# FauxFaux/quadrs

Hardware: AMD Instinct MI355X
Metric: Msamples/s through shift->FIR->FFT chain (higher is better)
Workload: dtype f32

## Files before the change

### quadrs_amd/csrc/qd_chain.h

```cpp
#pragma once

#include "qd_device.h"
#include "qd_geometry.h"

namespace qd {

#ifdef QD_STAMP
#define QD_STAMP_DECL unsigned long long st_prev = 0, st_acc[8] = {0, 0, 0, 0, 0, 0, 0, 0}, st_row[4] = {0, 0, 0, 0}; unsigned st_tiles = 0;
#define QD_STAMP_ROW(k) do { unsigned long long t_; asm volatile("s_memtime %0\n\ts_waitcnt lgkmcnt(0)" : "=s"(t_) :: "memory"); st_row[k] += t_ - st_prev; st_acc[0] += t_ - st_prev; st_prev = t_; } while (0)
#define QD_STAMP_START() do { asm volatile("s_memtime %0\n\ts_waitcnt lgkmcnt(0)" : "=s"(st_prev) :: "memory"); } while (0)
#define QD_STAMP_AT(k) do { unsigned long long t_; asm volatile("s_memtime %0\n\ts_waitcnt lgkmcnt(0)" : "=s"(t_) :: "memory"); st_acc[k] += t_ - st_prev; st_prev = t_; } while (0)
#define QD_STAMP_FLUSH() do { if (P.stamps && (threadIdx.x & 63) == 0 && threadIdx.x < 1024) { unsigned w_ = threadIdx.x >> 6; for (int k_ = 0; k_ < 8; ++k_) atomicAdd(&P.stamps[w_ * 8 + k_], st_acc[k_]); if (w_ == 1) for (int k_ = 0; k_ < 4; ++k_) atomicAdd(&P.stamps[129 + k_], st_row[k_]); if (w_ == 0) for (int k_ = 0; k_ < 4; ++k_) atomicAdd(&P.stamps[133 + k_], st_row[k_]); if (w_ == 0) atomicAdd(&P.stamps[128], (unsigned long long)st_tiles); } } while (0)
#define QD_STAMP_TILE() do { ++st_tiles; } while (0)
#else
#define QD_STAMP_DECL
#define QD_STAMP_START()
#define QD_STAMP_AT(k)
#define QD_STAMP_FLUSH()
#define QD_STAMP_TILE()
#define QD_STAMP_ROW(k)
#endif

#ifdef QD_DEVELOP
#define QD_DBG(P, bit) (((P).dbg & (bit)) != 0)
// ... 535 lines not shown
        }
    };
    auto load_h1 = [&](uint32_t j0, float *hh) {
        const float4 *hp = reinterpret_cast<const float4 *>(h + j0);
#pragma unroll
        for (int v = 0; v < BS / 4; ++v) {
            const float4 q = hp[v];
            hh[4 * v + 0] = q.x; hh[4 * v + 1] = q.y; hh[4 * v + 2] = q.z; hh[4 * v + 3] = q.w;
        }
    };
    auto load_h = [&](uint32_t blk, float (*hh)[BS]) {
#pragma unroll
        for (int r = 0; r < R; ++r) load_h1(blk * BS - r * D, hh[r]);
    };
    bool lane_trunc = false;
#pragma unroll
    for (int r = 0; r < R; ++r) lane_trunc |= jmax[r] < T;
    const bool need_snap = __builtin_amdgcn_ballot_w64(lane_trunc) != 0;
    auto snap_check = [&](int r, uint32_t j0) {
        if (need_snap && j0 >= T / 2 + D && ((j0 - T / 2) % D) == 0) {
            if (jmax[r] == j0) { sr[r] = ar[r]; si[r] = ai[r]; }
        }
    };
    auto mac_int = [&](uint32_t blk, const float2 *x, const float (*hh)[BS]) {
#pragma unroll
        for (int r = 0; r < R; ++r) snap_check(r, blk * BS - r * D);
#pragma unroll
        for (int i = 0; i < BS; ++i) {
#pragma unroll
            for (int r = 0; r < R; ++r) {
                ar[r] = ar[r] + x[i].x * hh[r][i];
                ai[r] = ai[r] + x[i].y * hh[r][i];
            }
        }
    };
    auto mac_edge = [&](uint32_t blk, const float2 *x) {
#pragma unroll
        for (int r = 0; r < R; ++r) {
            const int32_t j0 = (int32_t)(blk * BS) - r * (int32_t)D;
            if (j0 >= 0 && j0 < (int32_t)T) {
                snap_check(r, (uint32_t)j0);
                float hh[BS];
                load_h1((uint32_t)j0, hh);
#pragma unroll
                for (int i = 0; i < BS; ++i) {
                    ar[r] = ar[r] + x[i].x * hh[i];
                    ai[r] = ai[r] + x[i].y * hh[i];
                }
            }
        }
    };
    constexpr uint32_t P = (R - 1) * D / BS, E = T / BS;
    static_assert(E > P + 2, "filter too short for the register-tiled FIR");
    constexpr uint32_t P2 = P + ((E - P) & 1);
    float2 xa[BS], xb[BS];
    float ha[R][BS], hb[R][BS];
#pragma unroll
    for (uint32_t blk = 0; blk < P2; ++blk) {
        load_x(blk, xa);
        if (blk < P) mac_edge(blk, xa); else { load_h(blk, ha); mac_int(blk, xa, ha); }
    }
    load_x(P2, xa); load_h(P2, ha);
    for (uint32_t blk = P2; blk + 2 < E; blk += 2) {
        load_x(blk + 1, xb); load_h(blk + 1, hb);
        mac_int(blk, xa, ha);
        __builtin_amdgcn_sched_barrier(0);
        load_x(blk + 2, xa); load_h(blk + 2, ha);
        mac_int(blk + 1, xb, hb);
        __builtin_amdgcn_sched_barrier(0);
    }
    load_x(E - 1, xb); load_h(E - 1, hb);
    mac_int(E - 2, xa, ha);
    load_x(E, xa);
    mac_int(E - 1, xb, hb);
#pragma unroll
    for (uint32_t blk = E; blk < NB; ++blk) {
        if (blk > E) load_x(blk, xa);
        mac_edge(blk, xa);
    }
#pragma unroll
    for (int r = 0; r < R; ++r) { full[r] = make_float2(ar[r], ai[r]); snap[r] = make_float2(sr[r], si[r]); }
}

template <class GeoT>
__device__ __forceinline__ float fir_comp(const float *xp, uint32_t jmax, const float *h, float *snap_out = nullptr) {
    constexpr uint32_t D = GeoT::D, Dp = GeoT::Dp, T = GeoT::T, b = GeoT::b0;
    constexpr uint32_t PRE = (8 - b % 8) % 8, NBLK = (T - PRE) / 8, TAIL = (T - PRE) % 8;
    constexpr uint32_t CPOS = (T / 2 + 8 * D - PRE) % 8;
    static_assert(D % 8 == 0 && NBLK >= 3, "component-split FIR geometry");
    float acc = 0.f, snap = 0.f;
    auto cand = [&](uint32_t jj) -> bool { return jj >= T / 2 + D && jj < T && ((jj - T / 2) % D) == 0; };
    auto xoff = [&](uint32_t t) -> uint32_t { return 2 * ((t / D) * Dp + (t % D)); };
#pragma unroll
    for (uint32_t i = 0; i < PRE; ++i) {
        if (cand(i)) { if (jmax == i) snap = acc; }
        acc = acc + xp[xoff(b + i)] * h[i];
    }
    float xa[8], xb[8], ha[8], hb[8];
    auto load = [&](uint32_t m, float *x, float *hh) {
        const uint32_t t = b + PRE + 8 * m;
        const float *pp = xp + xoff(t);
#pragma unroll
        for (int i = 0; i < 8; ++i) x[i] = pp[2 * i];
        if constexpr (PRE % 4 == 0) {
            const float4 *hp = reinterpret_cast<const float4 *>(h + PRE + 8 * m);
            const float4 h0 = hp[0], h1 = hp[1];
            hh[0] = h0.x; hh[1] = h0.y; hh[2] = h0.z; hh[3] = h0.w; hh[4] = h1.x; hh[5] = h1.y; hh[6] = h1.z; hh[7] = h1.w;
        } else {
#pragma unroll
            for (int i = 0; i < 8; ++i) hh[i] = h[PRE + 8 * m + i];
        }
    };
    auto mac = [&](uint32_t m, const float *x, const float *hh) {
#pragma unroll
        for (uint32_t i = 0; i < 8; ++i) {
            if (i == CPOS) { const uint32_t jj = PRE + 8 * m + i; if (cand(jj) && jmax == jj) snap = acc; }
            acc = acc + x[i] * hh[i];
        }
    };
    constexpr uint32_t NPAIR = NBLK / 2;
    load(0, xa, ha);
    auto pair = [&](uint32_t m) {
        load(m + 1, xb, hb);
        mac(m, xa, ha);
        asm volatile("" : "+v"(acc));
        __builtin_amdgcn_sched_barrier(0);
        load(m + 2, xa, ha);
        mac(m + 1, xb, hb);
        asm volatile("" : "+v"(acc));
        __builtin_amdgcn_sched_barrier(0);
    };
    if constexpr (NPAIR <= 16) {
#pragma unroll
        for (uint32_t m = 0; m + 2 < 2 * NPAIR; m += 2) pair(m);
    } else {
#pragma unroll 1
        for (uint32_t m = 0; m + 2 < 2 * NPAIR; m += 2) pair(m);
    }
    load(2 * NPAIR - 1, xb, hb);
    mac(2 * NPAIR - 2, xa, ha);
    if constexpr (NBLK % 2) load(NBLK - 1, xa, ha);
    mac(2 * NPAIR - 1, xb, hb);
    if constexpr (NBLK % 2) mac(NBLK - 1, xa, ha);
#pragma unroll
    for (uint32_t i = 0; i < TAIL; ++i) {
        const uint32_t jj = PRE + 8 * NBLK + i;
        if (cand(jj)) { if (jmax == jj) snap = acc; }
        acc = acc + xp[xoff(b + jj)] * h[jj];
    }
    if (snap_out) { *snap_out = snap; return acc; }
    return jmax < T ? snap : acc;
}

template <class GeoT>
__device__ __forceinline__ float2 fir_pair(const float2 *rowp , uint32_t jmax, const float *h, float2 *snap_out = nullptr) {
    constexpr uint32_t D = GeoT::D, Dp = GeoT::Dp, T = GeoT::T, b = GeoT::b0, NB = T / 4;
    constexpr int PF = 3;
    static_assert(GeoT::kPad == 2 && T % 4 == 0 && b % 2 == 0 && D % 4 == 0 && NB > (uint32_t)PF, "packed FIR geometry");
#if defined(QD_FIR_ABL) && (QD_FIR_ABL & 4)
    if (snap_out) *snap_out = rowp[1];
    return rowp[0];
#endif
    v2f acc = {0.f, 0.f}, snap = {0.f, 0.f};
    auto cand = [&](uint32_t jj) -> bool { return jj >= T / 2 + D && jj < T && ((jj - T / 2) % D) == 0; };
    auto xoff = [&](uint32_t t) -> uint32_t { return (t / D) * Dp + (t % D); };
    float4 xa[PF], xb[PF], hh[PF];
    auto load = [&](uint32_t k, int slot) {
        const uint32_t t0 = b + 4 * k;
        xa[slot] = *reinterpret_cast<const float4 *>(rowp + xoff(t0));
        xb[slot] = *reinterpret_cast<const float4 *>(rowp + xoff(t0 + 2));
        hh[slot] = *reinterpret_cast<const float4 *>(h + 4 * k);
    };
#pragma unroll
    for (int k = 0; k < PF; ++k) load(k, k);
#pragma unroll
    for (uint32_t k = 0; k < NB; ++k) {
        const int slot = (int)(k % PF);
        if (cand(4 * k)) { if (jmax == 4 * k) snap = acc; }
        static_assert((T / 2) % 4 == 0, "snapshot taps sit on block boundaries");
        const v2f x0 = {xa[slot].x, xa[slot].y}, x1 = {xa[slot].z, xa[slot].w}, x2 = {xb[slot].x, xb[slot].y}, x3 = {xb[slot].z, xb[slot].w};
        const v2f h01 = {hh[slot].x, hh[slot].y}, h23 = {hh[slot].z, hh[slot].w};
        v2f p0, p1;
        if constexpr ((GeoT::kFlags & kGeoFastFma) != 0) {
            asm volatile("v_pk_fma_f32 %0, %1, %5, %0 op_sel_hi:[1,0,1]\n\t"
                         "v_pk_fma_f32 %0, %2, %5, %0 op_sel:[0,1,0] op_sel_hi:[1,1,1]\n\t"
                         "v_pk_fma_f32 %0, %3, %6, %0 op_sel_hi:[1,0,1]\n\t"
                         "v_pk_fma_f32 %0, %4, %6, %0 op_sel:[0,1,0] op_sel_hi:[1,1,1]"
                         : "+v"(acc)
                         : "v"(x0), "v"(x1), "v"(x2), "v"(x3), "v"(h01), "v"(h23));
        } else
        asm volatile("v_pk_mul_f32 %1, %3, %7 op_sel_hi:[1,0]\n\t"
                     "v_pk_mul_f32 %2, %4, %7 op_sel:[0,1] op_sel_hi:[1,1]\n\t"
                     "v_pk_add_f32 %0, %0, %1\n\t"
                     "v_pk_mul_f32 %1, %5, %8 op_sel_hi:[1,0]\n\t"
                     "v_pk_add_f32 %0, %0, %2\n\t"
                     "v_pk_mul_f32 %2, %6, %8 op_sel:[0,1] op_sel_hi:[1,1]\n\t"
                     "v_pk_add_f32 %0, %0, %1\n\t"
                     "v_pk_add_f32 %0, %0, %2"
                     : "+v"(acc), "=&v"(p0), "=&v"(p1)
                     : "v"(x0), "v"(x1), "v"(x2), "v"(x3), "v"(h01), "v"(h23));
        if (k + PF < NB) load(k + PF, slot);
        __builtin_amdgcn_sched_barrier(0);
    }
    if (snap_out) { *snap_out = make_float2(snap.x, snap.y); return make_float2(acc.x, acc.y); }
    const v2f r = jmax < T ? snap : acc;
    return make_float2(r.x, r.y);
}

template <class GeoT, int TURN>
__device__ __forceinline__ void fir_tiled2_pk(const float2 *lanep, const float *h, float2 *full, const uint32_t *jm, float2 *snap) {
    constexpr uint32_t D = GeoT::D, T = GeoT::T, c = GeoT::c;
    constexpr uint32_t L = D + T, NB = L / 4, HB = T / 4, LAG = D / 4;
    constexpr bool kReTap = LAG > 4;
    constexpr int PF = 3, NS = kReTap ? PF : PF + (int)LAG + 1;

    static_assert(GeoT::kFirTile == 2 && GeoT::PD == 2 * D && GeoT::pshift != 0xffffffffu && GeoT::kPad == 2, "two-output packed FIR: layout");
    static_assert(D % 4 == 0 && T % 4 == 0 && c % 4 == 0 && (T / 2) % 4 == 0 && NB > (uint32_t)PF && LAG >= 1 && LAG <= 8, "two-output packed FIR: geometry");
    v2f a0 = {0.f, 0.f}, a1 = {0.f, 0.f}, s0 = {0.f, 0.f}, s1 = {0.f, 0.f};
    const bool need_snap = __builtin_amdgcn_ballot_w64(jm[0] < T || jm[1] < T) != 0;
    auto cand = [&](uint32_t j) -> bool { return j >= T / 2 + D && j < T && ((j - T / 2) % D) == 0; };
    float4 xa[PF], xb[PF], hh[NS], gg[kReTap ? PF : 1];
    typedef float f4n __attribute__((ext_vector_type(4)));
    typedef __attribute__((address_space(3))) const f4n lds_f4;
    uint32_t hbase = (uint32_t)(uintptr_t)(__attribute__((address_space(3))) const void *)h;
    asm volatile("" : "+v"(hbase));
    const lds_f4 *hl = (const lds_f4 *)(uintptr_t)hbase;
    auto load = [&](uint32_t b) {
#if defined(QD_FIR_ABL) && (QD_FIR_ABL & 2)
        if (b >= (uint32_t)PF) return;
#endif
        const uint32_t t = c + 4 * b;
        const float2 *pp = lanep + (t + GeoT::kPad * (t >> GeoT::pshift));
        xa[b % PF] = *reinterpret_cast<const float4 *>(pp);
        xb[b % PF] = *reinterpret_cast<const float4 *>(pp + 2);
        if (b < HB) { const f4n q = hl[b]; hh[b % NS] = make_float4(q.x, q.y, q.z, q.w); }
        if constexpr (kReTap) { if (b >= LAG) { const f4n q = hl[b - LAG]; gg[b % PF] = make_float4(q.x, q.y, q.z, q.w); } }
    };
#pragma unroll
    for (int b = 0; b < PF; ++b) load(b);
#pragma clang loop unroll(full)
    for (uint32_t b = 0; b < NB; ++b) {
        const float4 A = xa[b % PF], B = xb[b % PF];
        const v2f x0 = {A.x, A.y}, x1 = {A.z, A.w}, x2 = {B.x, B.y}, x3 = {B.z, B.w};
        v2f t0, t1, t2, t3;
        if constexpr (TURN >= 0) { if ((b % 8) == 0) { if (((b / 8) & 1u) != (uint32_t)TURN) __builtin_amdgcn_s_setprio(2); else __builtin_amdgcn_s_setprio(1); } }
        if ((b < HB && cand(4 * b)) || (b >= LAG && cand(4 * (b - LAG)))) {
            if (need_snap) {
                if (b < HB && cand(4 * b)) { if (jm[0] == 4 * b) s0 = a0; }
                if (b >= LAG && cand(4 * (b - LAG))) { if (jm[1] == 4 * (b - LAG)) s1 = a1; }
            }
        }
#if defined(QD_FIR_ABL) && (QD_FIR_ABL & 1)
        {
            asm volatile("" :: "v"(x0), "v"(x3), "v"(hh[b % NS].x));
            if (b + PF < NB) load(b + PF);
            __builtin_amdgcn_sched_barrier(0);
            continue;
        }
#endif
        if (b >= LAG && b < HB) {
            const float4 H = hh[b % NS], G = kReTap ? gg[b % PF] : hh[(b - LAG) % NS];
            const v2f h01 = {H.x, H.y}, h23 = {H.z, H.w}, g01 = {G.x, G.y}, g23 = {G.z, G.w};
            if constexpr ((GeoT::kFlags & kGeoFastFma) != 0) {
                asm volatile("v_pk_fma_f32 %0, %2, %6, %0 op_sel_hi:[1,0,1]\n\t"
                             "v_pk_fma_f32 %1, %2, %8, %1 op_sel_hi:[1,0,1]\n\t"
                             "v_pk_fma_f32 %0, %3, %6, %0 op_sel:[0,1,0] op_sel_hi:[1,1,1]\n\t"
                             "v_pk_fma_f32 %1, %3, %8, %1 op_sel:[0,1,0] op_sel_hi:[1,1,1]\n\t"
                             "v_pk_fma_f32 %0, %4, %7, %0 op_sel_hi:[1,0,1]\n\t"
                             "v_pk_fma_f32 %1, %4, %9, %1 op_sel_hi:[1,0,1]\n\t"
                             "v_pk_fma_f32 %0, %5, %7, %0 op_sel:[0,1,0] op_sel_hi:[1,1,1]\n\t"
                             "v_pk_fma_f32 %1, %5, %9, %1 op_sel:[0,1,0] op_sel_hi:[1,1,1]"
                             : "+v"(a0), "+v"(a1)
                             : "v"(x0), "v"(x1), "v"(x2), "v"(x3), "v"(h01), "v"(h23), "v"(g01), "v"(g23));
            } else
            asm volatile("v_pk_mul_f32 %2, %6, %10 op_sel_hi:[1,0]\n\t"
                         "v_pk_mul_f32 %3, %6, %12 op_sel_hi:[1,0]\n\t"
                         "v_pk_mul_f32 %4, %7, %10 op_sel:[0,1] op_sel_hi:[1,1]\n\t"
                         "v_pk_add_f32 %0, %0, %2\n\t"
                         "v_pk_mul_f32 %5, %7, %12 op_sel:[0,1] op_sel_hi:[1,1]\n\t"
                         "v_pk_add_f32 %1, %1, %3\n\t"
                         "v_pk_mul_f32 %2, %8, %11 op_sel_hi:[1,0]\n\t"
                         "v_pk_add_f32 %0, %0, %4\n\t"
                         "v_pk_mul_f32 %3, %8, %13 op_sel_hi:[1,0]\n\t"
                         "v_pk_add_f32 %1, %1, %5\n\t"
                         "v_pk_mul_f32 %4, %9, %11 op_sel:[0,1] op_sel_hi:[1,1]\n\t"
                         "v_pk_add_f32 %0, %0, %2\n\t"
                         "v_pk_mul_f32 %5, %9, %13 op_sel:[0,1] op_sel_hi:[1,1]\n\t"
                         "v_pk_add_f32 %1, %1, %3\n\t"
                         "v_pk_add_f32 %0, %0, %4\n\t"
                         "v_pk_add_f32 %1, %1, %5"
                         : "+v"(a0), "+v"(a1), "=&v"(t0), "=&v"(t1), "=&v"(t2), "=&v"(t3)
                         : "v"(x0), "v"(x1), "v"(x2), "v"(x3), "v"(h01), "v"(h23), "v"(g01), "v"(g23));
        } else {
            const float4 H = b < HB ? hh[b % NS] : (kReTap ? gg[b % PF] : hh[(b - LAG) % NS]);
            const v2f h01 = {H.x, H.y}, h23 = {H.z, H.w};
            v2f &acc = b < HB ? a0 : a1;
            if constexpr ((GeoT::kFlags & kGeoFastFma) != 0) {
                asm volatile("v_pk_fma_f32 %0, %1, %5, %0 op_sel_hi:[1,0,1]\n\t"
                             "v_pk_fma_f32 %0, %2, %5, %0 op_sel:[0,1,0] op_sel_hi:[1,1,1]\n\t"
                             "v_pk_fma_f32 %0, %3, %6, %0 op_sel_hi:[1,0,1]\n\t"
                             "v_pk_fma_f32 %0, %4, %6, %0 op_sel:[0,1,0] op_sel_hi:[1,1,1]"
                             : "+v"(acc)
                             : "v"(x0), "v"(x1), "v"(x2), "v"(x3), "v"(h01), "v"(h23));
            } else
            asm volatile("v_pk_mul_f32 %1, %3, %7 op_sel_hi:[1,0]\n\t"
                         "v_pk_mul_f32 %2, %4, %7 op_sel:[0,1] op_sel_hi:[1,1]\n\t"
                         "v_pk_add_f32 %0, %0, %1\n\t"
                         "v_pk_mul_f32 %1, %5, %8 op_sel_hi:[1,0]\n\t"
                         "v_pk_add_f32 %0, %0, %2\n\t"
                         "v_pk_mul_f32 %2, %6, %8 op_sel:[0,1] op_sel_hi:[1,1]\n\t"
                         "v_pk_add_f32 %0, %0, %1\n\t"
                         "v_pk_add_f32 %0, %0, %2"
                         : "+v"(acc), "=&v"(t0), "=&v"(t1)
                         : "v"(x0), "v"(x1), "v"(x2), "v"(x3), "v"(h01), "v"(h23));
        }
        if (b + PF < NB) load(b + PF);
        __builtin_amdgcn_sched_barrier(0);
    }
    full[0] = make_float2(a0.x, a0.y);
    full[1] = make_float2(a1.x, a1.y);
    snap[0] = make_float2(s0.x, s0.y);
    snap[1] = make_float2(s1.x, s1.y);
}

template <class GeoT>
__device__ __forceinline__ float2 fir_prefix(const float2 *raw, uint32_t t0, uint32_t jmax, const float *h) {
    constexpr uint32_t T = GeoT::T;
    float ar = 0.f, ai = 0.f;
    uint32_t jhi = jmax;
#pragma unroll
    for (int off = 32; off >= 1; off >>= 1) { const uint32_t o = (uint32_t)__shfl_xor((int)jhi, off); jhi = o > jhi ? o : jhi; }
// ... 1165 lines not shown
template <> struct SparkSwz<8, 4> { static constexpr uint32_t m[4] = {0x50, 0x20, 0x0, 0x0}; };
template <> struct SparkSwz<64, 1> { static constexpr uint32_t m[4] = {0x40, 0x90, 0x20, 0x40}; };
template <> struct SparkSwz<128, 1> { static constexpr uint32_t m[4] = {0x8, 0x10, 0x20, 0x40}; };
template <> struct SparkSwz<32, 1> { static constexpr uint32_t m[4] = {0x8, 0x10, 0x20, 0x40}; };
template <> struct SparkSwz<16, 1> { static constexpr uint32_t m[4] = {0x10, 0x20, 0x40, 0x80}; };
template <> struct SparkSwz<256, 1> { static constexpr uint32_t m[4] = {0x40, 0x90, 0x20, 0x40}; };
template <class SZ> struct SparkSwzFn {
    static constexpr uint32_t mask_off(uint32_t off) {
        uint32_t r = 0;
        for (uint32_t d = 1; d <= 4; ++d) if ((SZ::m[d - 1] >> (d + off)) & 1u) r |= 1u << d;
        return r;
    }
    static __device__ __forceinline__ constexpr uint32_t delta(uint32_t p) {
        constexpr uint32_t k1 = mask_off(1), k2 = mask_off(2), k3 = mask_off(3), k4 = mask_off(4), k5 = mask_off(5), k6 = mask_off(6), k7 = mask_off(7), k8 = mask_off(8);
        return ((p >> 1) & k1) ^ ((p >> 2) & k2) ^ ((p >> 3) & k3) ^ ((p >> 4) & k4) ^ ((p >> 5) & k5) ^ ((p >> 6) & k6) ^ ((p >> 7) & k7) ^ ((p >> 8) & k8);
    }
};

typedef float spark_f2n __attribute__((ext_vector_type(2)));
typedef float spark_f4n __attribute__((ext_vector_type(4)));
typedef __attribute__((address_space(3))) spark_f2n spark_lds_f2;
typedef __attribute__((address_space(3))) spark_f4n spark_lds_f4;
__device__ __forceinline__ float2 spark_ld2(uint32_t a) { const spark_f2n v = *(const spark_lds_f2 *)(uintptr_t)a; return make_float2(v.x, v.y); }
__device__ __forceinline__ void spark_st2(uint32_t a, float2 v) { *(spark_lds_f2 *)(uintptr_t)a = spark_f2n{v.x, v.y}; }

template <class GeoT, uint32_t TS, uint32_t SPL, int PART = 3 , bool RT = false >
__device__ __forceinline__ void spark_fft_swz(const ChainParams &P, const float2 *twl, uint32_t fb , uint32_t lane_in,
                                              uint32_t n_win = TS / GeoT::W) {
    using SZ = SparkSwzFn<SparkSwz<GeoT::W, SPL>>;
    constexpr uint32_t base = GeoT::base_len, lb = GeoT::log_base, layers = GeoT::layers;
    static_assert(base == 8 || base == 16, "spark_fft_swz: W >= 8");
    uint32_t lo = lane_in;
    asm volatile("" : "+v"(lo));
    auto wsync = [] { __builtin_amdgcn_fence(__ATOMIC_ACQ_REL, "wavefront"); __builtin_amdgcn_wave_barrier(); };
    constexpr uint32_t n_task = TS / base;
    const uint32_t n_task_rt = n_win << (GeoT::logW - lb);
    if constexpr ((PART & 1) != 0) {
#pragma unroll
    for (uint32_t k = 0; k < (n_task + 63) / 64; ++k) {
        const uint32_t t = lo + 64 * k;
        if (RT ? t < n_task_rt : (n_task % 64 == 0 || t < n_task)) {
            const uint32_t r0 = t << lb, a0 = fb + ((r0 ^ SZ::delta(r0)) << 3);
            float2 v[base];
#pragma unroll
            for (uint32_t q = 0; q < base / 2; ++q) {
                const spark_f4n pc = *(const spark_lds_f4 *)(uintptr_t)(a0 ^ (16 * q));
                v[2 * q] = make_float2(pc.x, pc.y); v[2 * q + 1] = make_float2(pc.z, pc.w);
            }
            if constexpr (base == 16) bf16(v, P.tw16_1, P.tw16_2, P.tw16_3, P.root2); else bf8(v, P.root2);
            uint32_t a1 = a0;
            asm volatile("" : "+v"(a1));
#pragma unroll
            for (uint32_t q = 0; q < base / 2; ++q)
                *(spark_lds_f4 *)(uintptr_t)(a1 ^ (16 * q)) = spark_f4n{v[2 * q].x, v[2 * q].y, v[2 * q + 1].x, v[2 * q + 1].y};
        }
    }
    }
    uint32_t cols = base, log_cols = lb, tw_off = 0;
    const uint32_t n_bf_rt = n_win << (GeoT::logW - 2);
    if constexpr ((PART & 2) != 0) {
#pragma unroll
    for (uint32_t l = 0; l < layers; ++l) {
        wsync();
        float2 tc1 = make_float2(0.f, 0.f), tc2 = tc1, tc3 = tc1;
        if (cols <= 64) { const uint32_t i = lo & (cols - 1); tc1 = twl[tw_off + 3 * i]; tc2 = twl[tw_off + 3 * i + 1]; tc3 = twl[tw_off + 3 * i + 2]; }
#pragma unroll
        for (uint32_t k = 0; k < (TS / 4 + 63) / 64; ++k) {
            const uint32_t t = lo + 64 * k, chunk = t >> log_cols, i = t & (cols - 1);
            if (RT ? t >= n_bf_rt : ((TS / 4) % 64 != 0 && t >= TS / 4)) continue;
            const uint32_t p0 = chunk * 4 * cols + i, b0 = fb + ((p0 ^ SZ::delta(p0)) << 3);
            uint32_t dp[4];
#pragma unroll
            for (uint32_t q = 0; q < 4; ++q) {
                const uint32_t qc = q * cols, lo_q = (qc ^ SZ::delta(qc)) & 31u, hi_q = qc & ~31u;
                dp[q] = (b0 ^ (lo_q << 3)) + (hi_q << 3);
            }
            float2 t1 = tc1, t2 = tc2, t3 = tc3;
            if (cols > 64) { t1 = twl[tw_off + 3 * i]; t2 = twl[tw_off + 3 * i + 1]; t3 = twl[tw_off + 3 * i + 2]; }
            float2 s0 = spark_ld2(dp[0]);
            float2 s1 = cmul(spark_ld2(dp[1]), t1);
            float2 s2 = cmul(spark_ld2(dp[2]), t2);
            float2 s3 = cmul(spark_ld2(dp[3]), t3);
            bf4(s0, s1, s2, s3);
            spark_st2(dp[0], s0); spark_st2(dp[1], s1); spark_st2(dp[2], s2); spark_st2(dp[3], s3);
        }
        tw_off += 3 * cols; cols *= 4; log_cols += 2;
    }
    }
    wsync();
}


template <int FMT, class GeoT, int PT_ = kPipe3Prod>
struct Pipe3S {
    static_assert(PT_ == 256 || PT_ == 512, "producer threads: 256 or 512");
    static constexpr Pipe3sRules K = pipe3s_rules(FmtTraits<FMT>::SPL, PT_, GeoT::R);
    static constexpr uint32_t SPL = K.SPL, ROW = K.ROW;
    static constexpr uint32_t W = GeoT::W, S = GeoT::S, D = GeoT::D, T = GeoT::T, G = GeoT::G, Dp = GeoT::Dp;
    static constexpr uint32_t N = K.N, RN = K.RN, GS = K.GS;
    static constexpr uint32_t c_half = GeoT::c, ntrunc = GeoT::kNtrunc;
    static constexpr uint32_t f0 = K.f0, RR = K.RR, RINGD = K.RINGD, MIRD = K.MIRD, ROWP = K.ROWP, RAW_ELEMS = K.RAW_ELEMS, DR = K.DR;
    static constexpr bool kOverlap = K.kOverlap, fir_ok = K.fir_ok, ok = K.ok, kWrite = K.kWrite;
    static_assert(!kWrite || !kOverlap, "the write sink's sub-blocks lie side by side");
    static constexpr uint32_t FBX_OFF = K.FBX_OFF, kLdsBytes = K.kLdsBytes;
    static constexpr uint32_t GH = K.GH;
    static constexpr bool kSwzFft = K.kSwzFft;
    static constexpr uint32_t kConsumerThreads = K.kConsumerThreads;
};

template <int FMT, int NCO, class GeoT, int RN_, int LB, int PT_ = kPipe3Prod>
__global__ __launch_bounds__(PT_ + ((GeoT::kFlags & kGeoWriteSink) ? 256 : 512), LB) void k_chain_pipe3s(const ChainParams P) {
    static_assert((GeoT::kFlags & kGeoWindow) == 0, "kGeoWindow: only k_chain applies the plan's window; this kernel would ignore it");
    using FT = FmtTraits<FMT>;
    using Vec = typename FT::Vec;
    using K = Pipe3S<FMT, GeoT, PT_>;
    constexpr int SPL = FT::SPL;
    constexpr bool HAS_SHIFT = NCO != 0;
    static_assert(K::ok && (uint32_t)RN_ == K::RN, "streaming three-stage kernel: geometry");
    constexpr bool kWrite = K::kWrite;
    constexpr uint32_t PT = PT_, NTHR = PT_ + K::kConsumerThreads, PW = PT_ / 64;
    constexpr uint32_t W = K::W, S = K::S, D = K::D, T = K::T, G = K::G, Dp = K::Dp, logW = GeoT::logW;
    constexpr uint32_t ROW = K::ROW, ROWB = ROW * FT::BPS, VECB = SPL * FT::BPS, RN = K::RN, RR = K::RR, GS = K::GS, DR = K::DR;
    const GeoT geo(P);

    extern __shared__ __attribute__((aligned(16))) char smem[];
    float2 *raw = reinterpret_cast<float2 *>(smem);
    float2 *dec = raw + K::RAW_ELEMS, *trc = dec + DR;
    float2 *fbx = raw + K::FBX_OFF;
    float2 *twl = fbx + 2 * (size_t)G * W;
    float *tapl = reinterpret_cast<float *>(kWrite ? raw + K::RAW_ELEMS : twl + W);
    if (P.lds_dyn < K::kLdsBytes) return;

    const uint32_t tid = threadIdx.x;
    const uint32_t wave = __builtin_amdgcn_readfirstlane(tid >> 6);
    {
        if constexpr (!kWrite) {
            const uint32_t n_tw = W - geo.base_len;
            for (uint32_t i = tid; i < n_tw; i += NTHR) twl[i] = P.tw[i];
        }
        for (uint32_t i = tid; i < T; i += NTHR) tapl[i] = P.taps[i];
    }
    __syncthreads();

    const uint64_t n_tiles = (P.n_windows + G - 1) / G;
    const uint64_t base_cnt = n_tiles / gridDim.x, rem = n_tiles % gridDim.x;
    const uint64_t t_lo = (uint64_t)blockIdx.x * base_cnt + (blockIdx.x < rem ? blockIdx.x : rem);
    const uint32_t n_steps = (uint32_t)(base_cnt + (blockIdx.x < rem ? 1u : 0u));
    if (n_steps == 0) return;
    const uint32_t n_iter = n_steps + (kWrite ? 2u : 4u);
    auto g_cnt_of = [&](uint64_t t) -> uint32_t {
        const uint64_t w0 = t * G, left = P.n_windows - w0;
        return left < G ? (uint32_t)left : G;
    };

    if (wave < PW) {
        LaneRot lr[SPL];
        if constexpr (HAS_SHIFT) {
#pragma unroll
            for (int u = 0; u < SPL; ++u) {
                const uint32_t j = tid * SPL + u;
                lr[u] = nco_lane_rot((double)j, P.jtab[j]);
            }
        }
        const uint32_t lane_pad = pad_index(geo, tid * SPL);
        typedef unsigned v4u_t __attribute__((ext_vector_type(4)));
        typedef unsigned v2u_t __attribute__((ext_vector_type(2)));
        const uint64_t n0 = (P.first_window + t_lo * G) * ((uint64_t)S * D);
        auto rsrc_of = [&](uint32_t step1) {
            const uint64_t ns = n0 + (uint64_t)step1 * K::N;
            const uint64_t end = P.src_first + P.src_count;
            const uint64_t left = ns < end ? (end - ns) * FT::BPS : 0;
            return __builtin_amdgcn_make_buffer_rsrc(const_cast<uint8_t *>(P.src) + (ns - P.src_first) * FT::BPS, 0,
                                                     left > 0xffffffffull ? 0xffffffffu : (uint32_t)left, 0x00020000);
        };
        Vec pf[RN];
        auto load_row = [&](const decltype(rsrc_of(0)) &rsrc, int i) {
            constexpr int aux = ct_load_aux(GeoT::kFlags);
            if constexpr (sizeof(Vec) == 16) {
                const v4u_t w = __builtin_amdgcn_raw_buffer_load_b128(rsrc, (int)(tid * VECB), (int)(i * ROWB), aux);
                pf[i].x = w.x; pf[i].y = w.y; pf[i].z = w.z; pf[i].w = w.w;
            } else {
                const v2u_t w = __builtin_amdgcn_raw_buffer_load_b64(rsrc, (int)(tid * VECB), (int)(i * ROWB), aux);
                pf[i].x = w.x; pf[i].y = w.y;
            }
        };
        double rt_touch = 0.0;
        TileGeo gl{};
        gl.tile_raw = ROW;
        __builtin_amdgcn_s_setprio(0);
        {
            const auto rsrc = rsrc_of(0);
#pragma unroll
            for (int i = 0; i < (int)RN; ++i) load_row(rsrc, i);
        }
        uint32_t slot0 = 0;
        for (uint32_t it = 0; it < n_iter; ++it) {
            if (it <= n_steps && !QD_DBG(P, 256)) {
                const uint32_t step1 = it;
                const uint32_t pf1 = it < n_steps ? it + 1 : it;
                const auto rsrc = rsrc_of(pf1);
                const uint64_t ns = n0 + (uint64_t)step1 * K::N;
                const_f64_p rows = (const_f64_p)(uintptr_t)(P.rowtab + (ns / ROW - P.rowtab_row0));
                if constexpr (HAS_SHIFT) {
                    uint32_t r = tid < RN ? tid : RN - 1;
                    asm volatile("" : "+v"(r));
                    rt_touch += P.rowtab[(n0 + (uint64_t)pf1 * K::N) / ROW - P.rowtab_row0 + r].c;
                }
                RowBase rb_next{};
                if constexpr (HAS_SHIFT) rb_next = load_rowbase_at(rows, 0);
#pragma unroll
                for (int i = 0; i < (int)RN; ++i) {
                    const Vec v = pf[i];
                    const RowBase rb = rb_next;
                    if constexpr (HAS_SHIFT) { if (i + 1 < (int)RN) rb_next = load_rowbase_at(rows, i + 1); }
                    uint32_t slot = slot0 + (uint32_t)i;
                    if (slot >= RR) slot -= RR;
                    float2 *dst = raw + (size_t)slot * K::ROWP;
                    float2 *mir = slot == 0 ? raw + (size_t)K::RINGD * Dp : nullptr;
                    process_row<FMT, PT, NCO, true>(P, geo, gl, 0, tid, v, rb, lr, lane_pad, nullptr, dst, mir, K::MIRD * D);
                    __builtin_amdgcn_sched_barrier(0);
                    load_row(rsrc, i);
                    __builtin_amdgcn_sched_barrier(0);
                }
                slot0 += RN;
                if (slot0 >= RR) slot0 -= RR;
            }
            __syncthreads();
        }
        if (P.dbg == 0xdeadbeefu) reinterpret_cast<double *>(P.out)[tid] = rt_touch;
    } else if (wave < PW + 4) {
        __builtin_amdgcn_s_setprio(2);
        constexpr uint32_t ntrunc = K::ntrunc;
        for (uint32_t it = 0; it < n_iter; ++it) {
            if (it >= 1 && it <= n_steps + 1) {
                const uint32_t q_lo = it == 1 ? 0u : K::f0 + (it - 2) * GS, cnt = it == 1 ? K::f0 : GS;
                uint32_t l = tid - PT;
                asm volatile("" : "+v"(l));
                if (l < cnt && !QD_DBG(P, 64)) {
                    const uint32_t q = q_lo + l;
                    uint32_t jmax = T;
                    if constexpr (kWrite) {
                        const uint64_t sub = P.first_window + t_lo * G + (q >> logW);
                        const uint32_t kb = ((uint32_t)sub & P.blk_sub_mask) * W + (q & (W - 1));
                        const uint32_t jm = (P.blk_len - kb) * D + T / 2;
                        if (jm < T) jmax = jm;
                    } else
                    if constexpr (K::kOverlap) {
                        if (q + ntrunc >= W) {
                            const uint32_t g = (q - (W - ntrunc)) / S, k = q - g * S;
                            if (k < W) { const uint32_t jm = (W - k) * D + T / 2; if (jm < T) jmax = jm; }
                        }
                    } else {
                        const uint32_t k = q & (W - 1);
                        const uint32_t jm = (W - k) * D + T / 2;
                        if (jm < T) jmax = jm;
                    }
                    const uint32_t drow = (q + geo.a0) % K::RINGD;
                    const float2 *rowp = raw + (size_t)drow * Dp;
                    float2 snap = make_float2(0.f, 0.f);
                    typedef const float __attribute__((address_space(3))) *lds_f32_p;
                    uint32_t taps_off = (uint32_t)(uintptr_t)(lds_f32_p)tapl;
                    asm volatile("" : "+v"(taps_off));
                    const float *taps_v = (const float *)(lds_f32_p)(uintptr_t)taps_off;
                    const float2 full = fir_pair<GeoT>(rowp, jmax, taps_v, &snap);
                    const uint32_t pos = q % DR;
                    if constexpr (kWrite) {
                        const uint64_t qa = (t_lo * G << logW) + q;
                        if (qa < (P.n_windows << logW))
                            reinterpret_cast<float2 *>(P.out)[((P.first_window - P.out_window0) << logW) + qa] = jmax < T ? snap : full;
                    } else
                    if constexpr (K::kOverlap) {
                        dec[pos] = full;
                        if (jmax < T) trc[pos] = snap;
                    } else {
                        dec[pos] = jmax < T ? snap : full;
                    }
                }
            }
            __syncthreads();
        }
    } else if constexpr (!kWrite) {
        __builtin_amdgcn_s_setprio(1);
        const uint32_t v = wave - (PW + 4);
        constexpr uint32_t GH = (G + 1) / 2;
        const uint32_t g0 = (v & 1u) * GH;
        uint32_t rot = 0;
        for (uint32_t it = 0; it < n_iter; ++it) {
            if (v < 2) {
                if (it >= 3 && it - 3 < n_steps) {
                    const uint32_t s = it - 3;
                    const uint32_t g_cnt = g_cnt_of(t_lo + s);
                    const uint32_t g1 = (g0 + GH < g_cnt) ? g0 + GH : g_cnt;
                    if (g0 < g1 && !QD_DBG(P, 128)) {
                        float2 *fbw = fbx + (size_t)(s & 1u) * G * W + (size_t)g0 * W;
                        uint32_t lane = tid & 63u;
                        asm volatile("" : "+v"(lane));
                        constexpr uint32_t log_width = 2 * GeoT::layers;
                        const uint32_t n_o = (g1 - g0) << logW;
                        if constexpr (K::kSwzFft) {
                            using SZ = SparkSwzFn<SparkSwz<W, 1>>;
                            const uint32_t fb = (uint32_t)(uintptr_t)(__attribute__((address_space(3))) void *)fbw;
                            for (uint32_t o = lane; o < n_o; o += 64) {
                                const uint32_t gl_ = o >> logW, k = o & (W - 1);
                                uint32_t pos = rot + (g0 + gl_) * S + k;
                                pos = pos >= DR ? pos - DR : pos;
                                const bool tr = K::kOverlap && (W - k) * D + T / 2 < T;
                                const float2 val = dec[pos + (tr ? DR : 0u)];
                                const uint32_t xx = k & ((1u << log_width) - 1), yy = k >> log_width;
                                const uint32_t idx = (gl_ << logW) + yy + (rev4(xx, GeoT::layers) << GeoT::log_base);
                                spark_st2(fb + ((idx ^ SZ::delta(idx)) << 3), val);
                            }
                            __builtin_amdgcn_fence(__ATOMIC_ACQ_REL, "wavefront");
                            __builtin_amdgcn_wave_barrier();
                            spark_fft_swz<GeoT, K::GH * W, 1, 1, true>(P, twl, fb, lane, g1 - g0);
                        } else {
                        for (uint32_t o = lane; o < n_o; o += 64) {
                            const uint32_t gl_ = o >> logW, k = o & (W - 1);
                            uint32_t pos = rot + (g0 + gl_) * S + k;
                            pos = pos >= DR ? pos - DR : pos;
                            const bool tr = K::kOverlap && (W - k) * D + T / 2 < T;
                            const float2 val = dec[pos + (tr ? DR : 0u)];
                            const uint32_t xx = k & ((1u << log_width) - 1), yy = k >> log_width;
                            fbw[(gl_ << logW) + yy + (rev4(xx, geo.layers) << geo.log_base)] = val;
                        }
                        __builtin_amdgcn_fence(__ATOMIC_ACQ_REL, "wavefront");
                        __builtin_amdgcn_wave_barrier();
                        wave_fft_epilogue_fn<GeoT, 0, 1>(P, geo, twl, fbw, 0, g1 - g0, tid);
                        }
                    }
                }
                if (it >= 3) { rot += GS; rot = rot >= DR ? rot - DR : rot; }
            } else if (it >= 4) {
                const uint32_t s = it - 4;
                const uint64_t t = t_lo + s;
                const uint32_t g_cnt = g_cnt_of(t);
                const uint32_t g1 = (g0 + GH < g_cnt) ? g0 + GH : g_cnt;
                if (g0 < g1 && !QD_DBG(P, 128)) {
                    float2 *fbp = fbx + (size_t)(s & 1u) * G * W + (size_t)g0 * W;
                    if constexpr (K::kSwzFft) {
                        using SZ = SparkSwzFn<SparkSwz<W, 1>>;
                        const uint32_t fb = (uint32_t)(uintptr_t)(__attribute__((address_space(3))) void *)fbp;
                        uint32_t lane = tid & 63u;
                        asm volatile("" : "+v"(lane));
                        spark_fft_swz<GeoT, K::GH * W, 1, 2, true>(P, twl, fb, lane, g1 - g0);
                        const uint64_t wrel = P.first_window + t * G + g0 - P.out_window0;
                        const uint32_t n_out_s = (g1 - g0) << logW;
                        if (P.epi == 2) {
                            constexpr uint32_t KB = (K::GH * W + 63) / 64;
                            float nm[KB];
#pragma unroll
                            for (uint32_t k = 0; k < KB; ++k) { const uint32_t o = lane + 64 * k; nm[k] = o < n_out_s ? norm_ref(spark_ld2(fb + ((o ^ SZ::delta(o)) << 3))) : 0.f; }
                            __builtin_amdgcn_fence(__ATOMIC_ACQ_REL, "wavefront"); __builtin_amdgcn_wave_barrier();
                            float *nb = reinterpret_cast<float *>(fbp);
#pragma unroll
                            for (uint32_t k = 0; k < KB; ++k) { const uint32_t o = lane + 64 * k; if (o < n_out_s) nb[o] = nm[k]; }
                            __builtin_amdgcn_fence(__ATOMIC_ACQ_REL, "wavefront"); __builtin_amdgcn_wave_barrier();
                            for (uint32_t wl = lane; wl < g1 - g0; wl += 64) {
                                const float *q = nb + (wl << logW);
                                float first = 0.f, second = 0.f;
                                for (uint32_t k = 0; k < W / 2; ++k) first = first + q[k];
                                for (uint32_t k = W / 2; k < W; ++k) second = second + q[k];
                                reinterpret_cast<uint8_t *>(P.out)[wrel + wl] = first < second ? 0 : 1;
                            }
                        } else if (P.epi == 4) {
                            wave_mark_epilogue_fn<GeoT>(P, geo, [&](uint32_t o) { return spark_ld2(fb + ((o ^ SZ::delta(o)) << 3)); },
                                                        reinterpret_cast<uint8_t *>(P.out) + wrel, g1 - g0, lane);
                        } else {
                            float *outf = reinterpret_cast<float *>(P.out) + (wrel << logW);
                            uint8_t *outb = reinterpret_cast<uint8_t *>(P.out) + (wrel << logW);
                            for (uint32_t o = lane; o < n_out_s; o += 64) {
                                const uint32_t e = o ^ (W >> 1);
                                const float nm = norm_ref(spark_ld2(fb + ((e ^ SZ::delta(e)) << 3)));
                                if (P.epi == 0) outf[o] = nm;
                                else outb[o] = glyph_of<GeoT>(P, nm);
                            }
                        }
                    } else
                    wave_fft_epilogue_fn<GeoT, (GH * W + 63) / 64, 2>(P, geo, twl, fbp, P.first_window + t * G + g0, g1 - g0, tid);
                }
            }
            __syncthreads();
        }
    }
}


struct SparkWalk {
    uint64_t first, stride, end;
    __device__ __forceinline__ SparkWalk(uint64_t n_tiles, uint32_t wave) {
        constexpr uint32_t WPG = kThreads / 64;
        if ((gridDim.x & 7u) == 0 && n_tiles >= 64) {
            const uint64_t n8 = (n_tiles + 7) / 8, lo = (uint64_t)(blockIdx.x & 7u) * n8;
            first = lo + (uint64_t)(blockIdx.x >> 3) * WPG + wave;
            stride = (uint64_t)(gridDim.x >> 3) * WPG;
            end = lo + n8 < n_tiles ? lo + n8 : n_tiles;
            if (lo >= n_tiles) { first = n_tiles; end = n_tiles; }
        } else {
            first = (uint64_t)blockIdx.x * WPG + wave; stride = (uint64_t)gridDim.x * WPG; end = n_tiles;
        }
    }
};

template <class GeoT, bool F = GeoT::kFixed> struct W_CT_GE8 { static constexpr bool value = false; };
template <class GeoT> struct W_CT_GE8<GeoT, true> { static constexpr bool value = GeoT::W >= 8; };
static_assert(sizeof(LaneEntry) == kLaneEntryBytes, "the lane table's entry as qd_geometry.h sizes it");
constexpr uint32_t kSparkLaneLds = kSparkRow * kLaneEntryBytes / 8;
template <int FMT> struct SparkTraits {
    using FT = FmtTraits<FMT>;
    static constexpr uint32_t SPL = FT::SPL, CH = 64u * SPL, RQ = kSparkRow / CH;
};

template <int FMT, int NCO, class GeoT, int NCH, int LB, int EPI = -1 >
__global__ __launch_bounds__(kThreads, LB) void k_spark(const ChainParams P) {
    static_assert((GeoT::kFlags & kGeoWindow) == 0, "kGeoWindow: only k_chain applies the plan's window; this kernel would ignore it");
    using FT = FmtTraits<FMT>;
    using Vec = typename FT::Vec;
    using ST = SparkTraits<FMT>;
    constexpr int SPL = FT::SPL;
    constexpr bool HAS_SHIFT = NCO != 0;
    constexpr uint32_t CH = ST::CH, RQ = ST::RQ, TS = (uint32_t)NCH * CH, CHB = CH * FT::BPS, VECB = SPL * FT::BPS;
    static_assert(TS % kSparkRow == 0 && (NCH % RQ) == 0, "a tile is a whole number of NCO rows");
    const GeoT geo(P);
    const uint32_t W = geo.W, logW = geo.logW;
    const uint32_t G = TS >> logW;

    extern __shared__ __attribute__((aligned(16))) char smem[];
    float2 *twl = reinterpret_cast<float2 *>(smem);
    const uint32_t tid = threadIdx.x, lane = tid & 63u;
    const uint32_t wave = __builtin_amdgcn_readfirstlane(tid >> 6);
    constexpr bool kLdsLane = HAS_SHIFT && GeoT::kFixed;
    LaneEntry *jt = reinterpret_cast<LaneEntry *>(twl + (W < 32u ? 32u : W));
    float2 *fbw = twl + (W < 32u ? 32u : W) + (kLdsLane ? kSparkLaneLds : 0u) + (size_t)wave * TS;
    {
        const uint32_t n_tw = W - geo.base_len;
        for (uint32_t i = tid; i < n_tw; i += kThreads) twl[i] = P.tw[i];
        if constexpr (kLdsLane) { for (uint32_t i = tid; i < kSparkRow; i += kThreads) jt[i] = P.jtab[i]; }
    }
    __syncthreads();

    uint32_t pos[NCH * SPL];
    {
        const uint32_t log_width = 2 * geo.layers;
#pragma unroll
        for (int c = 0; c < NCH; ++c)
#pragma unroll
            for (int u = 0; u < SPL; ++u) {
                const uint32_t m = (uint32_t)c * CH + lane * SPL + (uint32_t)u, k = m & (W - 1);
                const uint32_t xx = k & ((1u << log_width) - 1), yy = k >> log_width;
                pos[c * SPL + u] = (m & ~(W - 1)) + yy + (rev4(xx, geo.layers) << geo.log_base);
            }
    }
    constexpr bool kLeanEpi = GeoT::kFixed && (EPI == 0 || EPI == 1 || EPI == 2);
    const uint32_t fb_off = (uint32_t)(uintptr_t)(__attribute__((address_space(3))) void *)fbw;
    if (kLeanEpi && (fb_off & 255u)) __builtin_trap();
// ... 551 lines not shown
```

Measured before the change: 652,100.

## Precompute FIR snapshot masks, carry ring offsets, and hoist FFT gather indexing

FIR lanes now compute jmax once per lane where the geometry allows. They pick the snapshot with ballot-derived SGPR masks and v_cndmask instead of per-lane compares, and they carry byte offsets into the raw and decimation rings using a single conditional subtract in place of modulo. The FFT gather for small W precomputes each lane's source and destination swizzled addresses once and walks them in unrolled rounds. This cuts per-iteration integer, division and modulo work on the FIR and FFT waves, at the cost of extra SGPR/VGPR state and static assumptions about how the ring wraps.

```diff
diff --git a/quadrs_amd/csrc/qd_chain.h b/quadrs_amd/csrc/qd_chain.h
--- a/quadrs_amd/csrc/qd_chain.h
+++ b/quadrs_amd/csrc/qd_chain.h
@@ -711,8 +711,18 @@
     return jmax < T ? snap : acc;
 }
 
+template <class GeoT> struct FirSnap {
+    static constexpr uint32_t first = GeoT::T / 2 + GeoT::D, N = GeoT::T > first ? (GeoT::T - first + GeoT::D - 1) / GeoT::D : 0;
+    uint64_t lanes[N > 0 ? N : 1];
+    __device__ __forceinline__ void set(uint32_t jmax) {
+#pragma unroll
+        for (uint32_t i = 0; i < N; ++i) lanes[i] = __builtin_amdgcn_ballot_w64(jmax == first + i * GeoT::D);
+    }
+};
+
 template <class GeoT>
-__device__ __forceinline__ float2 fir_pair(const float2 *rowp , uint32_t jmax, const float *h, float2 *snap_out = nullptr) {
+__device__ __forceinline__ float2 fir_pair(const float2 *rowp , uint32_t jmax, const float *h, float2 *snap_out = nullptr,
+                                           const FirSnap<GeoT> *snap_lanes = nullptr) {
     constexpr uint32_t D = GeoT::D, Dp = GeoT::Dp, T = GeoT::T, b = GeoT::b0, NB = T / 4;
     constexpr int PF = 3;
     static_assert(GeoT::kPad == 2 && T % 4 == 0 && b % 2 == 0 && D % 4 == 0 && NB > (uint32_t)PF, "packed FIR geometry");
@@ -735,7 +745,16 @@
 #pragma unroll
     for (uint32_t k = 0; k < NB; ++k) {
         const int slot = (int)(k % PF);
-        if (cand(4 * k)) { if (jmax == 4 * k) snap = acc; }
+        if (cand(4 * k)) {
+            if (snap_lanes) {
+                float sx = snap.x, sy = snap.y;
+                const float ax = acc.x, ay = acc.y;
+                asm volatile("v_cndmask_b32 %0, %0, %2, %4\n\t"
+                             "v_cndmask_b32 %1, %1, %3, %4"
+                             : "+v"(sx), "+v"(sy) : "v"(ax), "v"(ay), "s"(snap_lanes->lanes[(4 * k - FirSnap<GeoT>::first) / D]));
+                snap = v2f{sx, sy};
+            } else if (jmax == 4 * k) snap = acc;
+        }
         static_assert((T / 2) % 4 == 0, "snapshot taps sit on block boundaries");
         const v2f x0 = {xa[slot].x, xa[slot].y}, x1 = {xa[slot].z, xa[slot].w}, x2 = {xb[slot].x, xb[slot].y}, x3 = {xb[slot].z, xb[slot].w};
         const v2f h01 = {hh[slot].x, hh[slot].y}, h23 = {hh[slot].z, hh[slot].w};
@@ -2207,6 +2226,7 @@
         const uint64_t w0 = t * G, left = P.n_windows - w0;
         return left < G ? (uint32_t)left : G;
     };
+    auto wrap_once = [](uint32_t x, uint32_t ring) -> uint32_t { const uint32_t y = x - ring; return y < x ? y : x; };
 
     if (wave < PW) {
         LaneRot lr[SPL];
@@ -2286,50 +2306,71 @@
     } else if (wave < PW + 4) {
         __builtin_amdgcn_s_setprio(2);
         constexpr uint32_t ntrunc = K::ntrunc;
+        constexpr bool kJmaxOfLane = !kWrite && (!K::kOverlap || K::f0 + ntrunc >= W);
+        constexpr uint32_t ROWPB = Dp * 8, RINGB = K::RINGD * ROWPB, DRB = DR * 8;
+        static_assert(K::f0 + GeoT::a0 <= K::RINGD && 2 * GS + GeoT::a0 <= K::RINGD && 2 * GS <= DR && K::f0 <= GS, "FIR lanes: one conditional subtract wraps a carried ring offset");
+        auto jmax_of = [&](uint32_t q) -> uint32_t {
+            uint32_t jmax = T;
+            if constexpr (K::kOverlap) {
+                if (q + ntrunc >= W) {
+                    const uint32_t g = (q - (W - ntrunc)) / S, k = q - g * S;
+                    if (k < W) { const uint32_t jm = (W - k) * D + T / 2; if (jm < T) jmax = jm; }
+                }
+            } else {
+                const uint32_t k = q & (W - 1);
+                const uint32_t jm = (W - k) * D + T / 2;
+                if (jm < T) jmax = jm;
+            }
+            return jmax;
+        };
+        uint32_t l = tid - PT;
+        asm volatile("" : "+v"(l));
+        uint32_t row_b = (l + GeoT::a0) * ROWPB, pos_b = l * 8;
+        uint32_t jmax = T;
+        FirSnap<GeoT> snap_lanes;
+        if constexpr (kJmaxOfLane) { jmax = jmax_of(l); snap_lanes.set(jmax); }
         for (uint32_t it = 0; it < n_iter; ++it) {
             if (it >= 1 && it <= n_steps + 1) {
-                const uint32_t q_lo = it == 1 ? 0u : K::f0 + (it - 2) * GS, cnt = it == 1 ? K::f0 : GS;
-                uint32_t l = tid - PT;
-                asm volatile("" : "+v"(l));
+                const uint32_t cnt = it == 1 ? K::f0 : GS;
                 if (l < cnt && !QD_DBG(P, 64)) {
-                    const uint32_t q = q_lo + l;
-                    uint32_t jmax = T;
+                    [[maybe_unused]] uint32_t q = 0;
+                    if constexpr (!kJmaxOfLane) q = (it == 1 ? 0u : K::f0 + (it - 2) * GS) + l;
                     if constexpr (kWrite) {
                         const uint64_t sub = P.first_window + t_lo * G + (q >> logW);
                         const uint32_t kb = ((uint32_t)sub & P.blk_sub_mask) * W + (q & (W - 1));
                         const uint32_t jm = (P.blk_len - kb) * D + T / 2;
-                        if (jm < T) jmax = jm;
-                    } else
-                    if constexpr (K::kOverlap) {
-                        if (q + ntrunc >= W) {
-                            const uint32_t g = (q - (W - ntrunc)) / S, k = q - g * S;
-                            if (k < W) { const uint32_t jm = (W - k) * D + T / 2; if (jm < T) jmax = jm; }
-                        }
-                    } else {
-                        const uint32_t k = q & (W - 1);
-                        const uint32_t jm = (W - k) * D + T / 2;
-                        if (jm < T) jmax = jm;
+                        jmax = jm < T ? jm : T;
+                        snap_lanes.set(jmax);
+                    } else if constexpr (!kJmaxOfLane) {
+                        jmax = jmax_of(q);
+                        snap_lanes.set(jmax);
                     }
-                    const uint32_t drow = (q + geo.a0) % K::RINGD;
-                    const float2 *rowp = raw + (size_t)drow * Dp;
+                    const float2 *rowp = reinterpret_cast<const float2 *>(reinterpret_cast<const char *>(raw) + row_b);
                     float2 snap = make_float2(0.f, 0.f);
                     typedef const float __attribute__((address_space(3))) *lds_f32_p;
                     uint32_t taps_off = (uint32_t)(uintptr_t)(lds_f32_p)tapl;
                     asm volatile("" : "+v"(taps_off));
                     const float *taps_v = (const float *)(lds_f32_p)(uintptr_t)taps_off;
-                    const float2 full = fir_pair<GeoT>(rowp, jmax, taps_v, &snap);
-                    const uint32_t pos = q % DR;
+                    const float2 full = fir_pair<GeoT>(rowp, jmax, taps_v, &snap, &snap_lanes);
                     if constexpr (kWrite) {
                         const uint64_t qa = (t_lo * G << logW) + q;
                         if (qa < (P.n_windows << logW))
                             reinterpret_cast<float2 *>(P.out)[((P.first_window - P.out_window0) << logW) + qa] = jmax < T ? snap : full;
-                    } else
-                    if constexpr (K::kOverlap) {
-                        dec[pos] = full;
-                        if (jmax < T) trc[pos] = snap;
                     } else {
-                        dec[pos] = jmax < T ? snap : full;
+                        float2 *decp = reinterpret_cast<float2 *>(reinterpret_cast<char *>(dec) + pos_b);
+                        if constexpr (K::kOverlap) {
+                            decp[0] = full;
+                            if (jmax < T) decp[DR] = snap;
+                        } else {
+                            decp[0] = jmax < T ? snap : full;
+                        }
                     }
+                }
+                const uint32_t adv = it == 1 ? K::f0 : GS;
+                row_b = wrap_once(row_b + adv * ROWPB, RINGB);
+                pos_b = wrap_once(pos_b + adv * 8, DRB);
+                if constexpr (kJmaxOfLane) {
+                    if (it == 1) { jmax = jmax_of(K::f0 + l); snap_lanes.set(jmax); }
                 }
             }
             __syncthreads();
@@ -2340,6 +2381,22 @@
         constexpr uint32_t GH = (G + 1) / 2;
         const uint32_t g0 = (v & 1u) * GH;
         uint32_t rot = 0;
+        constexpr bool kRoundGather = K::kSwzFft && W <= 64;
+        constexpr uint32_t WPR = kRoundGather ? 64 / W : 1, NR = (GH * W + 63) / 64;
+        [[maybe_unused]] uint32_t gat_src = 0, gat_dst = 0;
+        [[maybe_unused]] const char *gat_ring = reinterpret_cast<const char *>(dec);
+        if constexpr (kRoundGather) {
+            using SZ = SparkSwzFn<SparkSwz<W, 1>>;
+            uint32_t lane = tid & 63u;
+            asm volatile("" : "+v"(lane));
+            constexpr uint32_t log_width = 2 * GeoT::layers;
+            const uint32_t gl_ = lane >> logW, k = lane & (W - 1);
+            const uint32_t xx = k & ((1u << log_width) - 1), yy = k >> log_width;
+            const uint32_t idx = (gl_ << logW) + yy + (rev4(xx, GeoT::layers) << GeoT::log_base);
+            gat_dst = (idx ^ SZ::delta(idx)) << 3;
+            gat_src = (gl_ * S + k) * 8;
+            if (K::kOverlap && (W - k) * D + T / 2 < T) gat_ring += DR * 8;
+        }
         for (uint32_t it = 0; it < n_iter; ++it) {
             if (v < 2) {
                 if (it >= 3 && it - 3 < n_steps) {
@@ -2355,6 +2412,18 @@
                         if constexpr (K::kSwzFft) {
                             using SZ = SparkSwzFn<SparkSwz<W, 1>>;
                             const uint32_t fb = (uint32_t)(uintptr_t)(__attribute__((address_space(3))) void *)fbw;
+                            if constexpr (kRoundGather) {
+                                const uint32_t p0 = gat_src + (rot + g0 * S) * 8, b0 = fb + gat_dst;
+#pragma unroll
+                                for (uint32_t j = 0; j < NR; ++j) {
+                                    if (64 * j >= n_o) break;
+                                    if (W == 64 || lane + 64 * j < n_o) {
+                                        const uint32_t p = wrap_once(p0 + j * (WPR * S * 8), DR * 8);
+                                        const float2 val = *reinterpret_cast<const float2 *>(gat_ring + p);
+                                        spark_st2((b0 ^ (SZ::delta(64 * j) << 3)) + 512 * j, val);
+                                    }
+                                }
+                            } else
                             for (uint32_t o = lane; o < n_o; o += 64) {
                                 const uint32_t gl_ = o >> logW, k = o & (W - 1);
                                 uint32_t pos = rot + (g0 + gl_) * S + k;
```

New measurement: 650,200 (median of 2 runs). No clear change (-0.3%).
